# yeyupiaoling/MASR

Measured on AMD Instinct MI355X. Metric: audio-seconds/sec (RTF^-1), conformer_streaming_fbank b32x10s, PCM->fbank->encoder->ctc_greedy->text, higher is better.
Workload: dtype f32; 1 GPU; configs[1]: conformer.yml streaming fbank, batch=32 synthetic 16 kHz 10 s utterances per GPU, ctc_greedy, random-init weights V=4233; global_batch=32, parallelism=dp1, world_size_observed=1, backend=none

## Files before the change

### masr_amd/csrc/common.h

```cpp
#pragma once
#include <hip/hip_runtime.h>
#include <stdint.h>

#include "lm_scorer.h"

#ifndef MASR_EXPERIMENTS
#define MASR_EXPERIMENTS 0
#endif

typedef float f32x4 __attribute__((ext_vector_type(4)));
typedef float f32x16 __attribute__((ext_vector_type(16)));

namespace masr {

struct LdsAttr {
    size_t granted[32] = {};
};
void ensure_dynamic_lds(const void* fn, size_t bytes, LdsAttr& st);
void note_launch_error(const char* what, hipError_t e);

#ifdef __HIPCC__
struct SeqRow {
    int b, t;
};
__device__ __forceinline__ SeqRow seq_row(int b0, int t0, int T, int lr) {
    SeqRow r{b0, t0 + lr};
    while (r.t >= T) {
        r.t -= T;
        ++r.b;
    }
    return r;
}

__device__ __forceinline__ float wave_sum_dpp(float v) {
#define MASR_DPP_F(x, ctrl, rows) \
    __builtin_bit_cast(float, __builtin_amdgcn_update_dpp(0, __builtin_bit_cast(int, (x)), (ctrl), (rows), 0xf, false))
    v += MASR_DPP_F(v, 0x111, 0xf);
    v += MASR_DPP_F(v, 0x112, 0xf);
    v += MASR_DPP_F(v, 0x114, 0xf);
    v += MASR_DPP_F(v, 0x118, 0xf);
    v += MASR_DPP_F(v, 0x142, 0xa);
    v += MASR_DPP_F(v, 0x143, 0xc);
#undef MASR_DPP_F
    return __builtin_bit_cast(float, __builtin_amdgcn_readlane(__builtin_bit_cast(int, v), 63));
}
#endif


enum GemmAct { ACT_NONE = 0, ACT_RELU = 1, ACT_SILU = 2 };
enum GemmAMode { A_PLAIN = 0, A_CONV2 = 1 };
enum GemmEpi { EPI_STD = 0, EPI_GLU = 1, EPI_SPLITK = 2 };

struct GemmArgs {
    const float* A;
    const float* W;
    const float* bias;
    float* C;
    const float* R;
    const int* lens;
    int M, N, K;
    int lda, ldc, ldr;
    int act;
    float alpha;
    int mask_tp;
    int bias_after_alpha;
    int T1, F1, T2, F2, Cc;
    int nsplit, ksplit;
    int skip_rps, skip_div;
    const float* Wp;
};

void launch_gemm(const GemmArgs& a, int amode, int epi, hipStream_t s);
void set_conv2_mid_fill(int pct);
void set_gemm_waves(int n);
void launch_pack_conv2_rows(const float* w, float* p, int K, hipStream_t s);
void launch_gemm_splitk(const GemmArgs& a, float* partial, int nsplit, hipStream_t s, int amode = A_PLAIN);
#if MASR_EXPERIMENTS
bool launch_gemm_bf16x3(const GemmArgs& a, int amode, hipStream_t s);
void set_gemm_bf16x3_waves(int n);
size_t ffn_x3_packed_elems(int dff);
void set_ffn_x3_rotation(int on);
void launch_pack_ffn_x3(const float* w1, const float* w2, unsigned short* p1, unsigned short* p2, int dff, hipStream_t s);
bool launch_ffn_x3(float* x, const float* lnw, const float* lnb, const unsigned short* p1, const float* b1,
                   const unsigned short* p2, const float* b2, int M, int dff, float eps, float scale, hipStream_t s);
#else
inline bool launch_gemm_bf16x3(const GemmArgs&, int, hipStream_t) { return false; }
inline void set_gemm_bf16x3_waves(int) {}
inline size_t ffn_x3_packed_elems(int) { return 0; }
inline void set_ffn_x3_rotation(int) {}
inline void launch_pack_ffn_x3(const float*, const float*, unsigned short*, unsigned short*, int, hipStream_t) {}
inline bool launch_ffn_x3(float*, const float*, const float*, const unsigned short*, const float*, const unsigned short*, const float*,
                          int, int, float, float, hipStream_t) { return false; }
#endif

void launch_layernorm(const float* x, const float* w, const float* b, float* y, int M, float eps,
                      int seq_t, int pad, const int* lens, hipStream_t s);
void set_conv1_nt(int on);
void launch_conv1(const float* feats, const float* mean, const float* istd, const float* w9c, const float* bias,
                  float* out, int B, int T, int F, int C, hipStream_t s);
void launch_dwconv_ln_silu(const float* g, const float* wkc, const float* bias, const float* lnw, const float* lnb,
                           float* out, int nseq, int Tq, int ktaps, float eps, hipStream_t s, const float* gconst = nullptr);
void launch_glu_const(const float* bias512, float* out256, hipStream_t s);
void launch_queue_spin(long long ticks, hipStream_t s);
void launch_queue_nop(hipStream_t s);
void launch_dwconv_bn_silu(const float* g, const float* wkc, const float* bias, const float* scale, const float* shift,
                           float* out, int nseq, int Tq, int ktaps, hipStream_t s, const float* gconst = nullptr);
void launch_dwconv_stride2_ln_silu(const float* g, const float* wkc, const float* bias, const float* lnw,
                                   const float* lnb, float* out, int nseq, int Tin, int ktaps, float eps, hipStream_t s);
void launch_avgpool2(const float* x, float* out, int B, int T, hipStream_t s);
void launch_time_reduce_dw(const float* x, const float* w5c, const float* bias, const int* lens, float* out, int B, int T,
                           int mstride, hipStream_t s);
void launch_recover_add(const float* saved, const float* y, float* x, int B, int T, int L, hipStream_t s);
void launch_softmax_argmax(float* logits, int M, int V, int ldv, int write_probs, int* idx, float* maxp, hipStream_t s);
void launch_ctc_collapse(const int* idx, const float* maxp, const int* nframes, int B, int Tp, int blank,
                         int* tokens, int* ntok, float* score, hipStream_t s);
struct PoolSeg {
    long src, dst;
    int n, pad_;
};
void launch_ctc_collapse_hist(const int* idx, const float* maxp, const int* nframes, const int* in_rows, int ld_in, int B, int Tp,
                              int blank, int* rows, hipStream_t s);
void launch_copy_segments(const float* src, float* dst, const float* src2, float* dst2, const PoolSeg* seg, int nseg,
                          int max_rows, int width, hipStream_t s);
void launch_ctc_collapse_rows(const int* idx, const float* maxp, const int* nframes, int B, int Tp, int blank, int* rows,
                              hipStream_t s);
void launch_topk_prune(const float* probs, int M, int V, int top_n, float cutoff_prob, int* out_idx, float* out_logp,
                       int* out_cnt, int blank, float* out_blank_lp, hipStream_t s);
void launch_argmax_rows(const float* probs, int M, int V, int* idx, float* maxp, hipStream_t s);
// ... 250 lines not shown
```

### masr_amd/csrc/engine.hip

```cpp
#include <math.h>
#include <stdio.h>
#include <stdlib.h>
#include <string.h>

#include <map>
#include <mutex>
#include <string>
#include <vector>

#include "../../include/masr_hip.h"
#include "common.h"

using namespace masr;
namespace masr {
int lm_device_view(masr_lm* lm, LmView* out);
bool lm_word_based(const masr_lm* lm);
}
extern "C" const char* masr_lm_last_error(void);

static thread_local std::string g_err;
static int fail(const std::string& m) {
    g_err = m;
    return 1;
}
// ... 283 lines not shown
    masr_engine* e;
    hipStream_t s;
    bool on;
    ProfScope(masr_engine* e_, hipStream_t s_, int kind, double flops) : e(e_), s(s_) {
        on = e->prof_kind != 0 && (e->prof_kind == kind || (e->prof_kind == PROF_GEMM && (kind == PROF_FFN1 || kind == PROF_CONV2 || kind == PROF_FFN_TAIL || kind == PROF_FFN_HEAD)));
        if (on && e->prof_stride > 1) on = (e->prof_seen++ % e->prof_stride) == 0;
        if (!on) return;
        if (e->prof_used == e->prof_events.size()) {
            hipEvent_t a, b;
            hipEventCreate(&a);
            hipEventCreate(&b);
            e->prof_events.push_back({a, b});
        }
        hipEventRecord(e->prof_events[e->prof_used].first, s);
        e->prof_flops += flops;
    }
    ~ProfScope() {
        if (!on) return;
        hipEventRecord(e->prof_events[e->prof_used].second, s);
        e->prof_used++;
    }
};

struct CallGuard {
    masr_engine* e;
    hipStream_t s;
    size_t n0;
    static size_t packed_count(const masr_engine* e) {
        return e->ffn_packed.size() + e->ffn_dual_packed.size() + e->x3_packed.size() + e->ffn16_packed.size() + e->conv2_packed.size();
    }
    CallGuard(masr_engine* e_, hipStream_t s_) : e(e_), s(s_), n0(packed_count(e_)) {
        if (!e->pack_pending) return;
        if (hipEventQuery(e->pack_ev) == hipSuccess) {
            e->pack_pending = false;
        } else {
            (void)hipGetLastError();
            if ((void*)s != e->pack_stream) (void)hipStreamWaitEvent(s, e->pack_ev, 0);
        }
    }
    ~CallGuard() {
        if (packed_count(e) == n0) return;
        if (!e->pack_ev && hipEventCreateWithFlags(&e->pack_ev, hipEventDisableTiming) != hipSuccess) return;
        if (hipEventRecord(e->pack_ev, s) == hipSuccess) {
            e->pack_stream = (void*)s;
            e->pack_pending = true;
        }
    }
};

static int g_ffn_dual = 0;
static int g_ffn_packed = 2;
static int g_ffn16 = 1;
static int g_conv2_rows = 1;
static int g_bf16x3 = 0;

void gemm(masr_engine* e, hipStream_t s, const float* A, int lda, const float* W, const float* bias, float* C, int ldc,
          int M, int N, int K, int act, float alpha, const float* R, int ldr, int kind = PROF_GEMM,
          const int* lens = nullptr, int mask_tp = 0) {
    GemmArgs a{};
    a.A = A; a.W = W; a.bias = bias; a.C = C; a.R = R; a.lens = lens;
    a.M = M; a.N = N; a.K = K; a.lda = lda; a.ldc = ldc; a.ldr = ldr;
    a.act = act; a.alpha = alpha; a.mask_tp = mask_tp;
    ProfScope ps(e, s, kind, 2.0 * M * (double)N * K);
    if (g_bf16x3 && launch_gemm_bf16x3(a, A_PLAIN, s)) return;
    launch_gemm(a, A_PLAIN, EPI_STD, s);
}

static int g_rowgemm_packed = 1;
const float* packed_rows_of(masr_engine* e, const float* W, int N, hipStream_t s) {
    auto it = e->ffn_packed.find(W);
    if (it == e->ffn_packed.end()) {
        const int Np = (N + 255) / 256 * 256;
        std::pair<DevBuf, DevBuf> pk;
        if (pk.first.ensure((size_t)Np * 256 * sizeof(float))) return nullptr;
        launch_pack_rows_pc(W, pk.first.as<float>(), Np, s, N);
        it = e->ffn_packed.emplace(W, pk).first;
    }
    return it->second.first.as<float>();
}

int packed_ffn_of(masr_engine* e, const float* w1, const float* w2, hipStream_t s, const float** p1, const float** p2) {
    const int d = e->cfg.d_model;
    auto it = e->ffn_packed.find(w1);
    if (it == e->ffn_packed.end()) {
        std::pair<DevBuf, DevBuf> pk;
        CHK(pk.first.ensure((size_t)e->cfg.d_ff * d * sizeof(float)));
        CHK(pk.second.ensure((size_t)e->cfg.d_ff * d * sizeof(float)));
        launch_pack_ffn_pc(w1, w2, pk.first.as<float>(), pk.second.as<float>(), e->cfg.d_ff, s);
        it = e->ffn_packed.emplace(w1, pk).first;
    }
    *p1 = it->second.first.as<float>();
    *p2 = it->second.second.as<float>();
    return 0;
}
static bool sqz_stage_supported(const masr_engine* e) {
    const int K = e->cfg.cnn_kernel;
    return e->cfg.d_model == 256 && e->cfg.d_ff % 128 == 0 && e->cfg.d_ff >= 256 && (K == 31 || K == 15);
}

void rowgemm(masr_engine* e, hipStream_t s, int pro, int epi, const float* A, int lda, const float* lnw,
             const float* lnb, const float* W, const float* bias, float* C, int ldc, int M, int N, const float* R,
             int ldr, float alpha, const int* lens, int mask_tp, int seq_t, int pad, int* out_idx, float* out_maxp,
             int kind = PROF_GEMM, int mstride = 4, int out_seq_t = 0, int out_pad_l = 0, int out_pad_tot = 0,
             int plane_cols = 0, long plane_stride = 0, int a_seq_t = 0, int a_seq_stride = 0, const AttSeq* kv_seqs = nullptr,
             int kv_tq = 0) {
    RowGemmArgs a{};
// ... 601 lines not shown
            std::pair<DevBuf, DevBuf> pk;
            CHK(pk.first.ensure((size_t)dff * d * sizeof(float)));
            CHK(pk.second.ensure((size_t)dff * d * sizeof(float)));
            launch_pack_ffn16(w1, w2, pk.first.as<float>(), pk.second.as<float>(), dff, s);
            it = e->ffn16_packed.emplace(w1, pk).first;
        }
        if (want_tail) {
            ptail = *tail;
            CHK(p16(tail->W, tail->N, &ptail.W));
        }
        if (want_head) {
            phead = *head;
            CHK(p16(head->W, d, &phead.W));
        }
        const int done = launch_ffn16(e->x.as<float>(), lnw, lnb, it->second.first.as<float>(), b1, it->second.second.as<float>(), b2, M,
                                      dff, 1e-5f, scale, s, want_tail ? &ptail : nullptr, want_head ? &phead : nullptr);
        if (done < 0) return fail("ffn(): the 16-row FFN kernel rejected the launch");
        if (want_head && done != 4) return fail("ffn(): head stage was not launched");
        if (tail_done) *tail_done = done == 2;
        if (post_y) launch_layernorm(e->x.as<float>(), post_w, post_b, post_y, M, 1e-5f, 0, 0, nullptr, s);
        return 0;
    }
    if (packed && want_tail && tail->N % 256 == 0) {
        ptail = *tail;
        CHK(packed_rows(tail->W, tail->N, &ptail.W));
        tail = &ptail;
    }
    if (packed && want_head) {
        phead = *head;
        CHK(packed_rows(head->W, d, &phead.W));
        if (split_head) {
            CHK(e->xh.ensure((size_t)M * d * sizeof(float)));
            phead.xout = e->xh.as<float>();
        }
        head = &phead;
    }
    const int done = launch_ffn_fused(e->x.as<float>(), lnw, lnb, kw1, b1, kw2, b2, M, dff, 1e-5f, scale, affine,
                                      nsplit > 1 ? e->ffpart.as<float>() : nullptr, nsplit, s, post_y ? &post : nullptr,
                                      want_tail ? tail : nullptr, want_head ? head : nullptr, packed);
    if (done < 0) return fail("ffn(): launch rejected");
    if (want_head && !(done & 4)) return fail("ffn(): head stage was not launched");
    if (tail_done) *tail_done = done == 2;
    if (post_y && !(done & 1)) launch_layernorm(e->x.as<float>(), post_w, post_b, post_y, M, 1e-5f, 0, 0, nullptr, s);
    return 0;
}

static int g_hot_weights = 0;
static int g_embed_split = 1;
int embed(masr_engine* e, hipStream_t s, const float* feats, int nseq, int T, int* Tq_out, const int* skip_lens = nullptr) {
    const int d = e->cfg.d_model, F = e->cfg.n_mels, F1 = (F - 1) / 2, F2 = (F1 - 1) / 2;
    const int T1 = (T - 1) / 2, Tq = (T1 - 1) / 2;
    if (T < 7 || Tq <= 0) return fail("input too short for Conv2dSubsampling4 (need >= 7 frames)");
    const int M = nseq * Tq;
    CHK(e->x1.ensure((size_t)nseq * T1 * F1 * d * sizeof(float)));
    CHK(e->x2.ensure((size_t)M * F2 * d * sizeof(float)));
    CHK(e->x.ensure((size_t)M * d * sizeof(float)));
    launch_conv1(feats, e->cmvn_mean, e->cmvn_istd, e->conv1_w, e->conv1_b, e->x1.as<float>(), nseq, T, F, d, s);
    {
        GemmArgs a{};
        a.A = e->x1.as<float>(); a.W = e->conv2_w; a.bias = e->conv2_b; a.C = e->x2.as<float>();
        a.M = M * F2; a.N = d; a.K = 9 * d; a.ldc = d; a.act = ACT_RELU; a.alpha = 1.f;
        a.T1 = T1; a.F1 = F1; a.T2 = Tq; a.F2 = F2; a.Cc = d;
        if (skip_lens) { a.lens = skip_lens; a.skip_rps = Tq * F2; a.skip_div = F2; }
        ProfScope ps(e, s, PROF_CONV2, 2.0 * a.M * (double)a.N * a.K);
        const int tiles = ((a.M + 63) / 64) * ((a.N + 63) / 64);
        if (g_bf16x3 && tiles >= 640 && launch_gemm_bf16x3(a, A_CONV2, s)) {
        } else if (tiles < 640) {
            const int nsplit = std::min(8, std::max(2, 1280 / tiles));
            CHK(e->ffpart.ensure((size_t)nsplit * a.M * a.N * sizeof(float)));
            launch_gemm_splitk(a, e->ffpart.as<float>(), nsplit, s, A_CONV2);
        } else {
            if (g_conv2_rows && a.N == 256) {
                auto it = e->conv2_packed.find(e->conv2_w);
                if (it == e->conv2_packed.end()) {
                    std::pair<DevBuf, DevBuf> pk;
                    CHK(pk.first.ensure((size_t)a.N * a.K * sizeof(float)));
                    launch_pack_conv2_rows(e->conv2_w, pk.first.as<float>(), a.K, s);
                    it = e->conv2_packed.emplace(e->conv2_w, pk).first;
                }
                a.Wp = it->second.first.as<float>();
            }
            launch_gemm(a, A_CONV2, EPI_STD, s);
        }
    }
    {
        GemmArgs a{};
        a.A = e->x2.as<float>(); a.lda = F2 * d; a.W = e->embed_w; a.bias = e->embed_b; a.C = e->x.as<float>(); a.ldc = d;
        a.M = M; a.N = d; a.K = F2 * d; a.act = ACT_NONE; a.alpha = sqrtf((float)d);
        a.bias_after_alpha = e->cfg.model_kind == 1 ? 1 : 0;
        if (skip_lens) { a.lens = skip_lens; a.skip_rps = Tq; a.skip_div = 1; }
        ProfScope ps(e, s, PROF_GEMM, 2.0 * M * (double)d * F2 * d);
        const int tiles = ((M + 63) / 64) * ((d + 63) / 64);
        const long wide = (long)((M + 63) / 64) * ((d + 127) / 128);
        const long t128 = (long)((M + 127) / 128) * ((d + 127) / 128);
        if (g_bf16x3 && tiles >= 128 && launch_gemm_bf16x3(a, A_PLAIN, s)) {
        } else if (g_embed_split && tiles >= 128 && t128 >= 100 && t128 <= 128) {
            CHK(e->ffpart.ensure((size_t)4 * M * d * sizeof(float)));
            launch_gemm_splitk(a, e->ffpart.as<float>(), 4, s);
        } else if (g_embed_split && tiles >= 128 && wide >= 200 && wide <= 320) {
            CHK(e->ffpart.ensure((size_t)2 * M * d * sizeof(float)));
            launch_gemm_splitk(a, e->ffpart.as<float>(), 2, s);
        } else if (tiles < 128) {
            const int nsplit = std::min(F2 * d / 32, std::max(2, 256 / tiles));
            CHK(e->ffpart.ensure((size_t)nsplit * M * d * sizeof(float)));
            launch_gemm_splitk(a, e->ffpart.as<float>(), nsplit, s);
        } else {
            launch_gemm(a, A_PLAIN, EPI_STD, s);
        }
    }
    *Tq_out = Tq;
    return 0;
}

int ensure_layer_ws(masr_engine* e, int nseq, int Tq) {
    const int d = e->cfg.d_model, pad = e->cfg.cnn_kernel - 1;
    const size_t M = (size_t)nseq * Tq;
    CHK(e->ln.ensure(M * d * sizeof(float)));
    CHK(e->qkv.ensure(M * 3 * d * sizeof(float)));
    CHK(e->att.ensure(M * d * sizeof(float)));
    CHK(e->lnpad.ensure((size_t)nseq * (Tq + pad) * d * sizeof(float)));
    CHK(e->glu.ensure((size_t)nseq * (Tq + pad) * d * sizeof(float)));
    CHK(e->dwo.ensure(M * d * sizeof(float)));
    return 0;
}

int conv_module(masr_engine* e, hipStream_t s, const LayerW& w, const EncodeCtx& c, bool hist, int K = 0, int mstride = 4,
                bool pw1_done = false, bool pw2_later = false) {
    if (K <= 0) K = e->cfg.cnn_kernel;
    const int d = e->cfg.d_model, pad = K - 1;
    const int M = c.nseq * c.Tq, Mp = c.nseq * (c.Tq + pad);
    float* x = e->x.as<float>();
    if (pw1_done) {
    } else if (hist) {
        launch_layernorm(x, w.ln_conv_w, w.ln_conv_b, e->lnpad.as<float>(), M, 1e-5f, c.Tq, pad, c.lens, s);
        rowgemm(e, s, RG_PRO_PLAIN, RG_EPI_GLU, e->lnpad.as<float>(), d, nullptr, nullptr, w.pw1_w, w.pw1_b,
                e->glu.as<float>(), d, Mp, 2 * d, nullptr, 0, 1.f, nullptr, 0, 0, 0, nullptr, nullptr);
    } else {
        rowgemm(e, s, RG_PRO_LN_PAD, RG_EPI_GLU, x, d, w.ln_conv_w, w.ln_conv_b, w.pw1_w, w.pw1_b, e->glu.as<float>(), d,
                M, 2 * d, nullptr, 0, 1.f, c.lens, 0, c.Tq, 0, nullptr, nullptr, PROF_GEMM, mstride, c.Tq,
                e->cfg.causal ? pad : pad / 2, pad);
    }
    if (pw2_later) return 0;
    const float* gconst = (hist || !e->cfg.causal) ? nullptr : w.gconst;
    {
        RowGemmArgs a{};
        a.A = e->glu.as<float>(); a.lda = d; a.lnw = w.cln_w; a.lnb = w.cln_b; a.dw_w = w.dw_w; a.dw_b = w.dw_b; a.gconst = gconst;
        a.W = w.pw2_w; a.bias = w.pw2_b; a.C = x; a.ldc = d; a.R = x; a.ldr = d; a.M = M; a.N = d; a.alpha = 1.f; a.eps = 1e-5f;
        a.mstride = mstride; a.seq_t = c.Tq; a.pad = pad; a.lens = c.lens; a.mask_tp = c.lens ? c.Tq : 0;
        ProfScope ps(e, s, PROF_GEMM, 2.0 * M * (double)d * d);
// ... 1638 lines not shown
    if (lane == e->lane) return 0;
    EngineWs& active = *e;
    e->parked[e->lane] = active;
    active = e->parked[lane];
    e->parked[lane] = EngineWs();
    e->lane = lane;
    return 0;
}

int masr_side_stream(masr_engine* e, int32_t kind, void** stream_out) {
    if (!e || !stream_out) return fail("null argument");
    if (kind < 0 || kind >= MASR_SIDE_STREAMS)
        return fail("masr_side_stream: kind must be 0 / 1 (prefix search), 2 (preparation), 3 (copy) or 4 (second encoder lane)");
    SideStreams* ss = nullptr;
    if (side_streams_of(e->cfg.device_id, &ss)) return 1;
    *stream_out = (void*)ss->s[kind];
    return 0;
}

int masr_debug_set(masr_engine* e, int32_t key, int32_t value) {
    if (!e) return fail("null engine");
#if !MASR_EXPERIMENTS
    if (value != 0 && (key == 20 || key == 21 || key == 22 || key == 24 || key == 30 || key == 34 || key == 35))
        return fail("masr_debug_set: this key selects an experimental kernel that is not in this build (MASR_BUILD_EXPERIMENTS=1)");
#endif
    if (key == 1) set_ffn_variant(value);
    else if (key == 5) g_no_chain = value;
    else if (key == 6) set_rowgemm_small(value);
    else if (key == 7) set_attention_fewq(value);
    else if (key == 14) set_attention_fold(value);
    else if (key == 15) g_embed_split = value;
    else if (key == 19) g_hot_weights = value;
    else if (key == 20) g_bf16x3 = value;
    else if (key == 21) set_gemm_bf16x3_waves(value);
    else if (key == 22) set_ffn_x3_rotation(value);
    else if (key == 23) g_ffn_packed = value;
    else if (key == 24) g_ffn_dual = value;
    else if (key == 25) g_rowgemm_packed = value;
    else if (key == 26) set_attention_grouped_fold(value);
    else if (key == 27) g_ctc_fused_blocks = value;
    else if (key == 28) set_attention_fewq_wgs(value);
    else if (key == 29) g_few_rows_path = value;
    else if (key == 30) g_split_head = value;
    else if (key == 31) g_efficient_fused = value;
    else if (key == 32) g_beam_lm_cache = value;
    else if (key == 33) set_conv2_mid_fill(value);
    else if (key == 34) g_attn_chain = value;
    else if (key == 35) g_ffn_coop = value;
    else if (key == 36) g_sqz_fused_blocks = value;
    else if (key == 37) g_beam_narrow = value;
    else if (key == 38) e->skip_padding = value;
    else if (key == 39) g_ffn16 = value;
    else if (key == 40) g_conv2_rows = value;
    else if (key == 17) set_gemm_waves(value);
    else if (key == 18) set_conv1_nt(value);
    else if (key == 16) { e->prof_stride = value > 1 ? value : 1; e->prof_seen = 0; }
    else if (key == 8) g_no_ffn_tail = value;
    else if (key == 9) g_no_ffn_head = value;
    else if (key == 12) set_rowgemm_small_blocks(value);
    else if (key == 13) g_ffn_split_blocks = value;
    else if (key == 2) {
        if (value) {
            if (!e->beam_prof) {
                void* p = nullptr;
                HIPCHK(hipMalloc(&p, 16 * sizeof(long long)));
                e->owned.push_back(p);
                e->beam_prof = (long long*)p;
            }
        } else if (e->beam_prof) {
            long long h[16];
            HIPCHK(hipMemcpy(h, e->beam_prof, sizeof(h), hipMemcpyDeviceToHost));
            fprintf(stderr, "beam phases (cycles, last workgroup): setup+hash %lld  extensions %lld  prefixes+count %lld  select %lld  compact %lld\n",
                    h[0], h[1], h[2], h[3], h[4]);
            fprintf(stderr, "  narrow step (%lld frames): tables+candidates %lld  hash+contexts %lld  children+scorer table %lld  extensions %lld  "
                    "prefixes+select %lld  scan %lld  survivors %lld  new prefixes %lld\n", h[5], h[6], h[7], h[8], h[9], h[10], h[11], h[12], h[13]);
            if (h[15] > 0) fprintf(stderr, "  wide step (%lld frames): %.1f distinct scorer contexts per frame\n", h[15], (double)h[14] / (double)h[15]);
            e->beam_prof = nullptr;
        }
    }
    else return fail("unknown debug key");
    return 0;
}

int masr_profile_select(masr_engine* e, int32_t kind) {
    if (!e) return fail("null engine");
    e->prof_kind = kind;
    return 0;
}

int masr_profile_read(masr_engine* e, double* total_ms, int64_t* launches, double* flops, int32_t reset) {
    if (!e) return fail("null engine");
    ENTER(e);
    double tot = 0.0;
    for (size_t i = 0; i < e->prof_used; ++i) {
        HIPCHK(hipEventSynchronize(e->prof_events[i].second));
        float ms = 0.f;
        HIPCHK(hipEventElapsedTime(&ms, e->prof_events[i].first, e->prof_events[i].second));
        tot += ms;
    }
    if (total_ms) *total_ms = tot;
    if (launches) *launches = (int64_t)e->prof_used;
    if (flops) *flops = e->prof_flops;
    if (reset) {
        e->prof_used = 0;
        e->prof_flops = 0.0;
    }
// ... 5 lines not shown
```

### masr_amd/csrc/gemm_f32.hip

```cpp
#include "common.h"

namespace masr {

static constexpr int BK = 32;
static constexpr int LDP = 36;

__device__ __forceinline__ float silu_f(float x) { return x / (1.0f + expf(-x)); }
__device__ __forceinline__ float sigmoid_f(float x) { return 1.0f / (1.0f + expf(-x)); }

template <int BM, int BN, int WM, int WN, int AMODE, int EPI>
__global__ __launch_bounds__(64 * WM * WN) void gemm_f32_kernel(GemmArgs p) {
    static_assert(WM * WN == 4 || WM * WN == 8, "4 or 8 waves");
    constexpr int NT = 64 * WM * WN;
    constexpr int RPP = NT / 8;
    constexpr int TM = BM / WM / 32;
    constexpr int TN = BN / WN / 32;
    constexpr int AL = BM / RPP;
    constexpr int WL = BN / RPP;
    extern __shared__ __align__(16) float smem[];
    float* As = smem;
    float* Ws = smem + 2 * BM * LDP;

    const int tid = threadIdx.x;
    const int lane = tid & 63;
// ... 114 lines not shown
    const int ccol = lane & 31;
    const int rbase = 4 * (lane >> 5);
    if (EPI == EPI_SPLITK) {
        float* cp = p.C + (size_t)blockIdx.y * p.M * p.ldc;
#pragma unroll
        for (int n = 0; n < TN; ++n) {
            const int col = bn + wn * (BN / WN) + n * 32 + ccol;
            if (col >= p.N) continue;
#pragma unroll
            for (int m = 0; m < TM; ++m)
#pragma unroll
                for (int r = 0; r < 16; ++r) {
                    const int row = bm + wm * (BM / WM) + m * 32 + (r & 3) + 8 * (r >> 2) + rbase;
                    if (row < p.M) cp[(size_t)row * p.ldc + col] = acc[m][n][r];
                }
        }
    }
    if (EPI == EPI_STD) {
#pragma unroll
        for (int n = 0; n < TN; ++n) {
            const int col = bn + wn * (BN / WN) + n * 32 + ccol;
            if (col >= p.N) continue;
            const float bv = p.bias ? p.bias[col] : 0.f;
#pragma unroll
            for (int m = 0; m < TM; ++m) {
                float res[16];
#pragma unroll
                for (int r = 0; r < 16; ++r) {
                    const int row = min(bm + wm * (BM / WM) + m * 32 + (r & 3) + 8 * (r >> 2) + rbase, p.M - 1);
                    res[r] = p.R ? p.R[(size_t)row * p.ldr + col] : 0.f;
                }
#pragma unroll
                for (int r = 0; r < 16; ++r) {
                    const int row = bm + wm * (BM / WM) + m * 32 + (r & 3) + 8 * (r >> 2) + rbase;
                    float v = acc[m][n][r] + (p.bias_after_alpha ? 0.f : bv);
                    if (p.act == ACT_RELU) v = fmaxf(v, 0.f);
                    else if (p.act == ACT_SILU) v = silu_f(v);
                    if (p.mask_tp > 0) {
                        const int rc = min(row, p.M - 1);
                        const int b = rc / p.mask_tp, t = rc - b * p.mask_tp;
                        if (4 * t >= p.lens[b]) v = 0.f;
                    }
                    v = res[r] + v * p.alpha + (p.bias_after_alpha ? bv : 0.f);
                    if (row < p.M) p.C[(size_t)row * p.ldc + col] = v;
                }
            }
        }
    }
}

static constexpr int RB_BM = 64;
static constexpr int RB_N = 256;
static constexpr int RB_RING = 8;

__device__ __forceinline__ f32x4 rb_bufld(__amdgpu_buffer_rsrc_t rs, unsigned lane16, unsigned frag) {
    return __builtin_bit_cast(f32x4, __builtin_amdgcn_raw_buffer_load_b128(rs, lane16, frag * 1024u, 0));
}

__global__ __launch_bounds__(512) __attribute__((amdgpu_waves_per_eu(4))) void conv2_rows_kernel(GemmArgs p) {
    __shared__ __align__(16) float As[2][RB_BM * LDP];
    const int tid = threadIdx.x, lane = tid & 63;
    const int wave = __builtin_amdgcn_readfirstlane(tid >> 6);
    const int nbm = (p.M + RB_BM - 1) / RB_BM;
    int bid = blockIdx.x;
    if (p.skip_rps <= 0) {
        const int q = nbm / 8, r = nbm % 8, xcd = bid % 8, idx = bid / 8;
        bid = (xcd < r ? xcd * (q + 1) : r * (q + 1) + (xcd - r) * q) + idx;
    }
    const int bm = bid * RB_BM;
    if (p.skip_rps > 0 && p.lens) {
        const int span = min(bm + RB_BM, p.M) - 1 - bm;
        const int b0 = bm / p.skip_rps, r0 = bm - b0 * p.skip_rps;
        if (r0 + span < p.skip_rps && 4 * (r0 / p.skip_div) >= p.lens[b0]) return;
    }

    const int lrow = tid >> 3, lc4 = (tid & 7) * 4;
    const float* aptr;
    const bool aok = bm + lrow < p.M;
    {
        const int mm = aok ? bm + lrow : 0;
        const int f2 = mm % p.F2, bt = mm / p.F2, t2 = bt % p.T2, b = bt / p.T2;
        aptr = p.A + (((size_t)b * p.T1 + 2 * t2) * p.F1 + 2 * f2) * p.Cc + lc4;
    }
    auto load_a = [&](int kt) -> f32x4 {
        const int cb = kt / 9, pos = kt - 9 * cb;
        const int kh = pos / 3, kw = pos - 3 * kh;
        const size_t aoff = ((size_t)kh * p.F1 + kw) * p.Cc + (size_t)cb * BK;
        return aok ? *reinterpret_cast<const f32x4*>(aptr + aoff) : f32x4{0.f, 0.f, 0.f, 0.f};
    };
    float* const adst = &As[0][lrow * LDP + lc4];

    const int KT = p.K / BK;
    const __amdgpu_buffer_rsrc_t wrs =
        __builtin_amdgcn_make_buffer_rsrc(const_cast<float*>(p.Wp), 0, RB_N * p.K * (int)sizeof(float), 0x00020000);
    const unsigned lane16 = lane * 16;
    const unsigned wfrag0 = (unsigned)(wave * KT) * 4u;
    auto bld = [&](int kt, int g) -> f32x4 { return rb_bufld(wrs, lane16, wfrag0 + (unsigned)min(kt, KT - 1) * 4u + g); };

    f32x4 pre[RB_RING];
#pragma unroll
    for (int i = 0; i < RB_RING; ++i) pre[i] = bld(i >> 2, i & 3);
    f32x16 acc[2];
#pragma unroll
    for (int m = 0; m < 2; ++m)
#pragma unroll
        for (int r = 0; r < 16; ++r) acc[m][r] = 0.f;

    *reinterpret_cast<f32x4*>(adst) = load_a(0);
    __syncthreads();

    const int frow = lane & 31, fcol = (lane >> 5) * 4;
    const float* afrag = &As[0][frow * LDP + fcol];
    for (int kt0 = 0; kt0 < KT; kt0 += 2) {
#pragma unroll
        for (int j = 0; j < 2; ++j) {
            const int kt = kt0 + j;
            if (j == 1 && kt >= KT) break;
            f32x4 areg;
            if (kt + 1 < KT) areg = load_a(kt + 1);
            const float* Ab = afrag + j * RB_BM * LDP;
            f32x4 af[2] = {*reinterpret_cast<const f32x4*>(Ab), *reinterpret_cast<const f32x4*>(Ab + 32 * LDP)};
            __builtin_amdgcn_sched_barrier(0);
#pragma unroll
            for (int g = 0; g < BK / 8; ++g) {
                f32x4 an[2];
                if (g + 1 < BK / 8) {
                    an[0] = *reinterpret_cast<const f32x4*>(Ab + (g + 1) * 8);
                    an[1] = *reinterpret_cast<const f32x4*>(Ab + 32 * LDP + (g + 1) * 8);
                }
                __builtin_amdgcn_sched_barrier(0);
#pragma unroll
                for (int s = 0; s < 4; ++s)
#pragma unroll
                    for (int m = 0; m < 2; ++m)
                        acc[m] = __builtin_amdgcn_mfma_f32_32x32x2f32(af[m][s], pre[4 * j + g][s], acc[m], 0, 0, 0);
                __builtin_amdgcn_sched_barrier(0);
                pre[4 * j + g] = bld(kt + 2, g);
                __builtin_amdgcn_sched_barrier(0);
                if (g + 1 < BK / 8) {
                    af[0] = an[0];
                    af[1] = an[1];
                }
            }
            if (kt + 1 < KT) *reinterpret_cast<f32x4*>(adst + (j ^ 1) * RB_BM * LDP) = areg;
            __syncthreads();
        }
    }

    const int ccol = lane & 31;
    const int rbase = 4 * (lane >> 5);
    const int col = wave * 32 + ccol;
    const float bv = p.bias ? p.bias[col] : 0.f;
#pragma unroll
    for (int m = 0; m < 2; ++m) {
        float res[16];
#pragma unroll
        for (int r = 0; r < 16; ++r) {
            const int row = min(bm + m * 32 + (r & 3) + 8 * (r >> 2) + rbase, p.M - 1);
            res[r] = p.R ? p.R[(size_t)row * p.ldr + col] : 0.f;
        }
#pragma unroll
        for (int r = 0; r < 16; ++r) {
            const int row = bm + m * 32 + (r & 3) + 8 * (r >> 2) + rbase;
            float v = acc[m][r] + (p.bias_after_alpha ? 0.f : bv);
            if (p.act == ACT_RELU) v = fmaxf(v, 0.f);
            else if (p.act == ACT_SILU) v = silu_f(v);
            if (p.mask_tp > 0) {
                const int rc = min(row, p.M - 1);
                const int b = rc / p.mask_tp, t = rc - b * p.mask_tp;
                if (4 * t >= p.lens[b]) v = 0.f;
            }
            v = res[r] + v * p.alpha + (p.bias_after_alpha ? bv : 0.f);
            if (row < p.M) p.C[(size_t)row * p.ldc + col] = v;
        }
    }
}

__global__ __launch_bounds__(256) void pack_conv2_rows_kernel(const float* __restrict__ w, float* __restrict__ p, int K) {
    const size_t e = (size_t)blockIdx.x * 256 + threadIdx.x;
    if (e >= (size_t)RB_N * K) return;
    const int KT = K / BK;
    const int q = (int)(e & 3), lane = (int)((e >> 2) & 63);
    const size_t frag = e >> 8;
    const int g = (int)(frag & 3), kt = (int)((frag >> 2) % KT), wave = (int)((frag >> 2) / KT);
    p[e] = w[(size_t)(32 * wave + (lane & 31)) * K + kt * BK + 8 * g + 4 * (lane >> 5) + q];
}
void launch_pack_conv2_rows(const float* w, float* p, int K, hipStream_t s) {
    const size_t n = (size_t)RB_N * K;
    hipLaunchKernelGGL(pack_conv2_rows_kernel, dim3((unsigned)((n + 255) / 256)), dim3(256), 0, s, w, p, K);
}

static int g_gemm_waves = 8;
static int g_conv2_mid_fill = 50;
void set_conv2_mid_fill(int pct) { g_conv2_mid_fill = pct; }
void set_gemm_waves(int n) { g_gemm_waves = n; }

template <int BM, int BN, int WM, int WN, int AMODE, int EPI>
static void launch_t(const GemmArgs& a, hipStream_t s) {
    const int nbm = (a.M + BM - 1) / BM, nbn = (a.N + BN - 1) / BN;
    const size_t lds = (size_t)2 * (BM + BN) * LDP * sizeof(float);
    auto k = gemm_f32_kernel<BM, BN, WM, WN, AMODE, EPI>;
    static LdsAttr attr;
    ensure_dynamic_lds(reinterpret_cast<const void*>(k), lds, attr);
    hipLaunchKernelGGL(k, dim3(nbm * nbn, EPI == EPI_SPLITK ? a.nsplit : 1), dim3(64 * WM * WN), lds, s, a);
}

__global__ __launch_bounds__(256) void splitk_reduce_kernel(GemmArgs p, const float* __restrict__ partial, float* out) {
    const size_t i = (size_t)blockIdx.x * 256 + threadIdx.x;
    if (i >= (size_t)p.M * p.N) return;
    const int row = (int)(i / p.N), col = (int)(i - (size_t)row * p.N);
    float acc = 0.f;
    for (int sp = 0; sp < p.nsplit; ++sp) acc += partial[((size_t)sp * p.M + row) * p.N + col];
    const float bv = p.bias ? p.bias[col] : 0.f;
    float v = acc + (p.bias_after_alpha ? 0.f : bv);
    if (p.act == ACT_RELU) v = fmaxf(v, 0.f);
    else if (p.act == ACT_SILU) v = silu_f(v);
    const float r = p.R ? p.R[(size_t)row * p.ldr + col] : 0.f;
    out[(size_t)row * p.ldc + col] = r + v * p.alpha + (p.bias_after_alpha ? bv : 0.f);
}

void launch_gemm(const GemmArgs& a, int amode, int epi, hipStream_t s) {
    if (a.M <= 0 || a.N <= 0) return;
    if (amode == A_CONV2 && epi == EPI_SPLITK) {
        launch_t<64, 64, 2, 2, A_CONV2, EPI_SPLITK>(a, s);
        return;
    }
    if (amode == A_CONV2) {
        const long t128c = (long)((a.M + 127) / 128) * ((a.N + 127) / 128);
        const long rounds = (t128c + 511) / 512;
        const bool thin_tail = g_conv2_mid_fill > 0 && t128c >= 200 && t128c <= 1024 &&
                               (t128c - (rounds - 1) * 512) * 100 < (long)g_conv2_mid_fill * 512;
        if (t128c < 200) launch_t<64, 64, 2, 2, A_CONV2, EPI_STD>(a, s);
        else if (thin_tail) launch_t<64, 128, 2, 2, A_CONV2, EPI_STD>(a, s);
        else if (a.Wp && a.N == RB_N && a.K % BK == 0)
            hipLaunchKernelGGL(conv2_rows_kernel, dim3((unsigned)((a.M + RB_BM - 1) / RB_BM)), dim3(512), 0, s, a);
        else if (g_gemm_waves == 8) launch_t<128, 128, 2, 4, A_CONV2, EPI_STD>(a, s);
        else launch_t<128, 128, 2, 2, A_CONV2, EPI_STD>(a, s);
        return;
    }
    if (epi == EPI_SPLITK) {
        if (a.nsplit >= 4 && (long)((a.M + 127) / 128) * ((a.N + 127) / 128) >= 100) launch_t<128, 128, 2, 4, A_PLAIN, EPI_SPLITK>(a, s);
        else if ((long)((a.M + 63) / 64) * ((a.N + 127) / 128) >= 200) launch_t<64, 128, 2, 2, A_PLAIN, EPI_SPLITK>(a, s);
        else launch_t<64, 64, 2, 2, A_PLAIN, EPI_SPLITK>(a, s);
        return;
    }
    const long t128 = (long)((a.M + 127) / 128) * ((a.N + 127) / 128);
    const long t64 = (long)((a.M + 63) / 64) * ((a.N + 127) / 128);
    if (t128 >= 384) launch_t<128, 128, 2, 2, A_PLAIN, EPI_STD>(a, s);
    else if (t64 >= 200) launch_t<64, 128, 2, 2, A_PLAIN, EPI_STD>(a, s);
    else launch_t<64, 64, 2, 2, A_PLAIN, EPI_STD>(a, s);
}

void launch_gemm_splitk(const GemmArgs& a, float* partial, int nsplit, hipStream_t s, int amode) {
    if (a.M <= 0 || a.N <= 0) return;
    GemmArgs b = a;
    const int kts = a.K / BK;
    b.ksplit = (kts + nsplit - 1) / nsplit;
    b.nsplit = (kts + b.ksplit - 1) / b.ksplit;
    b.C = partial;
    b.ldc = a.N;
    launch_gemm(b, amode, EPI_SPLITK, s);
    GemmArgs r = a;
    r.nsplit = b.nsplit;
    hipLaunchKernelGGL(splitk_reduce_kernel, dim3((unsigned)(((size_t)a.M * a.N + 255) / 256)), dim3(256), 0, s, r, partial, a.C);
}

}
```

Before: 51970 audio-seconds/sec.

## Fuse conv1 into conv2 row kernel and reuse row kernel for embed split-K

The conv2 row-streaming kernel gains a fused mode: it computes conv1 (CMVN, 3x3 conv, bias, ReLU) on the fly from the raw fbank features held in LDS, so the large x1 intermediate is never written or read back from global memory. The same kernel gets a plain-A split-K mode, used for the embedding linear layer with a row-packed weight. This removes the x1 round trip and the separate conv1 launch, at the cost of extra per-tile ALU work and LDS use inside the conv2 kernel. Recomputing conv1 per 64-row tile also duplicates overlapping input work.

```diff
diff --git a/masr_amd/csrc/common.h b/masr_amd/csrc/common.h
--- a/masr_amd/csrc/common.h
+++ b/masr_amd/csrc/common.h
@@ -68,12 +68,15 @@
     int nsplit, ksplit;
     int skip_rps, skip_div;
     const float* Wp;
+    const float *feats, *mean, *istd, *c1w, *c1b;
+    int Tin, Fin;
 };
 
 void launch_gemm(const GemmArgs& a, int amode, int epi, hipStream_t s);
 void set_conv2_mid_fill(int pct);
 void set_gemm_waves(int n);
 void launch_pack_conv2_rows(const float* w, float* p, int K, hipStream_t s);
+bool gemm_conv2_rows(const GemmArgs& a);
 void launch_gemm_splitk(const GemmArgs& a, float* partial, int nsplit, hipStream_t s, int amode = A_PLAIN);
 #if MASR_EXPERIMENTS
 bool launch_gemm_bf16x3(const GemmArgs& a, int amode, hipStream_t s);
diff --git a/masr_amd/csrc/engine.hip b/masr_amd/csrc/engine.hip
--- a/masr_amd/csrc/engine.hip
+++ b/masr_amd/csrc/engine.hip
@@ -359,6 +359,8 @@
 static int g_ffn_packed = 2;
 static int g_ffn16 = 1;
 static int g_conv2_rows = 1;
+static int g_conv1_fused = 1;
+static int g_embed_rows = 1;
 static int g_bf16x3 = 0;
 
 void gemm(masr_engine* e, hipStream_t s, const float* A, int lda, const float* W, const float* bias, float* C, int ldc,
@@ -1066,34 +1068,41 @@
     const int T1 = (T - 1) / 2, Tq = (T1 - 1) / 2;
     if (T < 7 || Tq <= 0) return fail("input too short for Conv2dSubsampling4 (need >= 7 frames)");
     const int M = nseq * Tq;
-    CHK(e->x1.ensure((size_t)nseq * T1 * F1 * d * sizeof(float)));
     CHK(e->x2.ensure((size_t)M * F2 * d * sizeof(float)));
     CHK(e->x.ensure((size_t)M * d * sizeof(float)));
-    launch_conv1(feats, e->cmvn_mean, e->cmvn_istd, e->conv1_w, e->conv1_b, e->x1.as<float>(), nseq, T, F, d, s);
     {
         GemmArgs a{};
-        a.A = e->x1.as<float>(); a.W = e->conv2_w; a.bias = e->conv2_b; a.C = e->x2.as<float>();
+        a.W = e->conv2_w; a.bias = e->conv2_b; a.C = e->x2.as<float>();
         a.M = M * F2; a.N = d; a.K = 9 * d; a.ldc = d; a.act = ACT_RELU; a.alpha = 1.f;
         a.T1 = T1; a.F1 = F1; a.T2 = Tq; a.F2 = F2; a.Cc = d;
         if (skip_lens) { a.lens = skip_lens; a.skip_rps = Tq * F2; a.skip_div = F2; }
+        const int tiles = ((a.M + 63) / 64) * ((a.N + 63) / 64);
+        if (tiles >= 640 && g_conv2_rows && a.N == 256) {
+            auto it = e->conv2_packed.find(e->conv2_w);
+            if (it == e->conv2_packed.end()) {
+                std::pair<DevBuf, DevBuf> pk;
+                CHK(pk.first.ensure((size_t)a.N * a.K * sizeof(float)));
+                launch_pack_conv2_rows(e->conv2_w, pk.first.as<float>(), a.K, s);
+                it = e->conv2_packed.emplace(e->conv2_w, pk).first;
+            }
+            a.Wp = it->second.first.as<float>();
+            if (g_conv1_fused && !g_bf16x3 && gemm_conv2_rows(a)) {
+                a.feats = feats; a.mean = e->cmvn_mean; a.istd = e->cmvn_istd; a.c1w = e->conv1_w; a.c1b = e->conv1_b;
+                a.Tin = T; a.Fin = F;
+            }
+        }
+        if (!a.feats) {
+            CHK(e->x1.ensure((size_t)nseq * T1 * F1 * d * sizeof(float)));
+            launch_conv1(feats, e->cmvn_mean, e->cmvn_istd, e->conv1_w, e->conv1_b, e->x1.as<float>(), nseq, T, F, d, s);
+            a.A = e->x1.as<float>();
+        }
         ProfScope ps(e, s, PROF_CONV2, 2.0 * a.M * (double)a.N * a.K);
-        const int tiles = ((a.M + 63) / 64) * ((a.N + 63) / 64);
         if (g_bf16x3 && tiles >= 640 && launch_gemm_bf16x3(a, A_CONV2, s)) {
         } else if (tiles < 640) {
             const int nsplit = std::min(8, std::max(2, 1280 / tiles));
             CHK(e->ffpart.ensure((size_t)nsplit * a.M * a.N * sizeof(float)));
             launch_gemm_splitk(a, e->ffpart.as<float>(), nsplit, s, A_CONV2);
         } else {
-            if (g_conv2_rows && a.N == 256) {
-                auto it = e->conv2_packed.find(e->conv2_w);
-                if (it == e->conv2_packed.end()) {
-                    std::pair<DevBuf, DevBuf> pk;
-                    CHK(pk.first.ensure((size_t)a.N * a.K * sizeof(float)));
-                    launch_pack_conv2_rows(e->conv2_w, pk.first.as<float>(), a.K, s);
-                    it = e->conv2_packed.emplace(e->conv2_w, pk).first;
-                }
-                a.Wp = it->second.first.as<float>();
-            }
             launch_gemm(a, A_CONV2, EPI_STD, s);
         }
     }
@@ -1109,6 +1118,16 @@
         const long t128 = (long)((M + 127) / 128) * ((d + 127) / 128);
         if (g_bf16x3 && tiles >= 128 && launch_gemm_bf16x3(a, A_PLAIN, s)) {
         } else if (g_embed_split && tiles >= 128 && t128 >= 100 && t128 <= 128) {
+            if (g_embed_rows && d == 256 && (F2 * d) % 32 == 0) {
+                auto it = e->conv2_packed.find(e->embed_w);
+                if (it == e->conv2_packed.end()) {
+                    std::pair<DevBuf, DevBuf> pk;
+                    CHK(pk.first.ensure((size_t)a.N * a.K * sizeof(float)));
+                    launch_pack_conv2_rows(e->embed_w, pk.first.as<float>(), a.K, s);
+                    it = e->conv2_packed.emplace(e->embed_w, pk).first;
+                }
+                a.Wp = it->second.first.as<float>();
+            }
             CHK(e->ffpart.ensure((size_t)4 * M * d * sizeof(float)));
             launch_gemm_splitk(a, e->ffpart.as<float>(), 4, s);
         } else if (g_embed_split && tiles >= 128 && wide >= 200 && wide <= 320) {
@@ -2853,6 +2872,8 @@
     else if (key == 38) e->skip_padding = value;
     else if (key == 39) g_ffn16 = value;
     else if (key == 40) g_conv2_rows = value;
+    else if (key == 41) g_conv1_fused = value;
+    else if (key == 42) g_embed_rows = value;
     else if (key == 17) set_gemm_waves(value);
     else if (key == 18) set_conv1_nt(value);
     else if (key == 16) { e->prof_stride = value > 1 ? value : 1; e->prof_seen = 0; }
diff --git a/masr_amd/csrc/gemm_f32.hip b/masr_amd/csrc/gemm_f32.hip
--- a/masr_amd/csrc/gemm_f32.hip
+++ b/masr_amd/csrc/gemm_f32.hip
@@ -190,13 +190,20 @@
 static constexpr int RB_BM = 64;
 static constexpr int RB_N = 256;
 static constexpr int RB_RING = 8;
+static constexpr int RB_PP = 49;
+enum { RB_X1 = 0, RB_FUSED = 1, RB_PLAIN = 2 };
 
 __device__ __forceinline__ f32x4 rb_bufld(__amdgpu_buffer_rsrc_t rs, unsigned lane16, unsigned frag) {
     return __builtin_bit_cast(f32x4, __builtin_amdgcn_raw_buffer_load_b128(rs, lane16, frag * 1024u, 0));
 }
 
+__device__ constexpr int rb_tap(int g) { return g == 0 ? 0 : g == 1 ? 2 : g == 2 ? 4 : g == 3 ? 6 : 9; }
+
+template <int AM>
 __global__ __launch_bounds__(512) __attribute__((amdgpu_waves_per_eu(4))) void conv2_rows_kernel(GemmArgs p) {
+    constexpr int XS = AM == RB_FUSED ? 10 * RB_N + RB_BM * RB_PP : 4;
     __shared__ __align__(16) float As[2][RB_BM * LDP];
+    __shared__ __align__(16) float Xs[XS];
     const int tid = threadIdx.x, lane = tid & 63;
     const int wave = __builtin_amdgcn_readfirstlane(tid >> 6);
     const int nbm = (p.M + RB_BM - 1) / RB_BM;
@@ -211,24 +218,33 @@
         const int b0 = bm / p.skip_rps, r0 = bm - b0 * p.skip_rps;
         if (r0 + span < p.skip_rps && 4 * (r0 / p.skip_div) >= p.lens[b0]) return;
     }
+    const int KT = p.K / BK;
+    const int kt_lo = AM == RB_PLAIN ? (int)blockIdx.y * p.ksplit : 0;
+    const int kt_hi = AM == RB_PLAIN ? min(kt_lo + p.ksplit, KT) : KT;
 
     const int lrow = tid >> 3, lc4 = (tid & 7) * 4;
-    const float* aptr;
+    const float* aptr = nullptr;
     const bool aok = bm + lrow < p.M;
-    {
+    if (AM == RB_X1) {
         const int mm = aok ? bm + lrow : 0;
         const int f2 = mm % p.F2, bt = mm / p.F2, t2 = bt % p.T2, b = bt / p.T2;
         aptr = p.A + (((size_t)b * p.T1 + 2 * t2) * p.F1 + 2 * f2) * p.Cc + lc4;
+    } else if (AM == RB_PLAIN) {
+        aptr = p.A + (size_t)(aok ? bm + lrow : 0) * p.lda + lc4;
     }
     auto load_a = [&](int kt) -> f32x4 {
-        const int cb = kt / 9, pos = kt - 9 * cb;
-        const int kh = pos / 3, kw = pos - 3 * kh;
-        const size_t aoff = ((size_t)kh * p.F1 + kw) * p.Cc + (size_t)cb * BK;
+        size_t aoff;
+        if (AM == RB_PLAIN) {
+            aoff = (size_t)kt * BK;
+        } else {
+            const int cb = kt / 9, pos = kt - 9 * cb;
+            const int kh = pos / 3, kw = pos - 3 * kh;
+            aoff = ((size_t)kh * p.F1 + kw) * p.Cc + (size_t)cb * BK;
+        }
         return aok ? *reinterpret_cast<const f32x4*>(aptr + aoff) : f32x4{0.f, 0.f, 0.f, 0.f};
     };
     float* const adst = &As[0][lrow * LDP + lc4];
 
-    const int KT = p.K / BK;
     const __amdgpu_buffer_rsrc_t wrs =
         __builtin_amdgcn_make_buffer_rsrc(const_cast<float*>(p.Wp), 0, RB_N * p.K * (int)sizeof(float), 0x00020000);
     const unsigned lane16 = lane * 16;
@@ -237,25 +253,71 @@
 
     f32x4 pre[RB_RING];
 #pragma unroll
-    for (int i = 0; i < RB_RING; ++i) pre[i] = bld(i >> 2, i & 3);
+    for (int i = 0; i < RB_RING; ++i) pre[i] = bld(kt_lo + (i >> 2), i & 3);
+    __builtin_amdgcn_sched_barrier(0);
+
+    const float* const w1s = Xs;
+    const float* const xrow = Xs + 10 * RB_N + lrow * RB_PP;
+    if (AM == RB_FUSED) {
+        for (int i = tid; i < 9 * RB_N; i += 512) Xs[i] = p.c1w[i];
+        if (tid < RB_N) Xs[9 * RB_N + tid] = p.c1b[tid];
+        const int m = min(bm + lrow, p.M - 1);
+        const int f2 = m % p.F2, bt = m / p.F2, t2 = bt % p.T2, b = bt / p.T2;
+        const float* src = p.feats + ((size_t)b * p.Tin + 4 * t2) * p.Fin + 4 * f2;
+        for (int q = tid & 7; q < RB_PP; q += 8) {
+            const int dt = q / 7, df = q - 7 * dt, f = 4 * f2 + df;
+            Xs[10 * RB_N + lrow * RB_PP + q] = (src[dt * p.Fin + df] - p.mean[f]) * p.istd[f];
+        }
+    }
+    auto c1_rd = [&](int kt, int t, f32x4& w, float& x) {
+        const int cb = kt / 9, pos = kt - 9 * cb, kh = pos / 3, kw = pos - 3 * kh;
+        x = xrow[2 * kh * 7 + 2 * kw + (t / 3) * 7 + t % 3];
+        w = *reinterpret_cast<const f32x4*>(w1s + t * RB_N + 32 * cb + lc4);
+    };
+    auto c1_fma = [&](f32x4& c, const f32x4& w, float x) {
+#pragma unroll
+        for (int q = 0; q < 4; ++q) c[q] = fmaf(w[q], x, c[q]);
+    };
+    auto c1_bias = [&](int kt) -> f32x4 { return *reinterpret_cast<const f32x4*>(w1s + 9 * RB_N + 32 * (kt / 9) + lc4); };
+    auto c1_relu = [&](f32x4& c) {
+#pragma unroll
+        for (int q = 0; q < 4; ++q) c[q] = fmaxf(c[q], 0.f);
+    };
+
+    if (AM == RB_FUSED) {
+        __syncthreads();
+        f32x4 c = c1_bias(0);
+#pragma unroll
+        for (int t = 0; t < 9; ++t) {
+            f32x4 w;
+            float x;
+            c1_rd(0, t, w, x);
+            c1_fma(c, w, x);
+        }
+        c1_relu(c);
+        *reinterpret_cast<f32x4*>(adst) = c;
+    }
     f32x16 acc[2];
 #pragma unroll
     for (int m = 0; m < 2; ++m)
 #pragma unroll
         for (int r = 0; r < 16; ++r) acc[m][r] = 0.f;
 
-    *reinterpret_cast<f32x4*>(adst) = load_a(0);
+    if (AM != RB_FUSED) *reinterpret_cast<f32x4*>(adst) = load_a(kt_lo);
     __syncthreads();
 
     const int frow = lane & 31, fcol = (lane >> 5) * 4;
     const float* afrag = &As[0][frow * LDP + fcol];
-    for (int kt0 = 0; kt0 < KT; kt0 += 2) {
+    for (int kt0 = kt_lo; kt0 < kt_hi; kt0 += 2) {
 #pragma unroll
         for (int j = 0; j < 2; ++j) {
             const int kt = kt0 + j;
-            if (j == 1 && kt >= KT) break;
+            if (j == 1 && kt >= kt_hi) break;
+            const bool next = kt + 1 < kt_hi;
+            const int ktn = min(kt + 1, kt_hi - 1);
             f32x4 areg;
-            if (kt + 1 < KT) areg = load_a(kt + 1);
+            if (AM == RB_FUSED) areg = c1_bias(ktn);
+            else if (next) areg = load_a(kt + 1);
             const float* Ab = afrag + j * RB_BM * LDP;
             f32x4 af[2] = {*reinterpret_cast<const f32x4*>(Ab), *reinterpret_cast<const f32x4*>(Ab + 32 * LDP)};
             __builtin_amdgcn_sched_barrier(0);
@@ -266,6 +328,13 @@
                     an[0] = *reinterpret_cast<const f32x4*>(Ab + (g + 1) * 8);
                     an[1] = *reinterpret_cast<const f32x4*>(Ab + 32 * LDP + (g + 1) * 8);
                 }
+                constexpr int NTAP = 3;
+                f32x4 cw[NTAP];
+                float cx[NTAP];
+                if (AM == RB_FUSED) {
+#pragma unroll
+                    for (int t = rb_tap(g); t < rb_tap(g + 1); ++t) c1_rd(ktn, t, cw[t - rb_tap(g)], cx[t - rb_tap(g)]);
+                }
                 __builtin_amdgcn_sched_barrier(0);
 #pragma unroll
                 for (int s = 0; s < 4; ++s)
@@ -275,12 +344,17 @@
                 __builtin_amdgcn_sched_barrier(0);
                 pre[4 * j + g] = bld(kt + 2, g);
                 __builtin_amdgcn_sched_barrier(0);
+                if (AM == RB_FUSED) {
+#pragma unroll
+                    for (int t = rb_tap(g); t < rb_tap(g + 1); ++t) c1_fma(areg, cw[t - rb_tap(g)], cx[t - rb_tap(g)]);
+                }
                 if (g + 1 < BK / 8) {
                     af[0] = an[0];
                     af[1] = an[1];
                 }
             }
-            if (kt + 1 < KT) *reinterpret_cast<f32x4*>(adst + (j ^ 1) * RB_BM * LDP) = areg;
+            if (AM == RB_FUSED) c1_relu(areg);
+            if (next) *reinterpret_cast<f32x4*>(adst + (j ^ 1) * RB_BM * LDP) = areg;
             __syncthreads();
         }
     }
@@ -288,6 +362,17 @@
     const int ccol = lane & 31;
     const int rbase = 4 * (lane >> 5);
     const int col = wave * 32 + ccol;
+    if (AM == RB_PLAIN) {
+        float* cp = p.C + (size_t)blockIdx.y * p.M * p.ldc;
+#pragma unroll
+        for (int m = 0; m < 2; ++m)
+#pragma unroll
+            for (int r = 0; r < 16; ++r) {
+                const int row = bm + m * 32 + (r & 3) + 8 * (r >> 2) + rbase;
+                if (row < p.M) cp[(size_t)row * p.ldc + col] = acc[m][r];
+            }
+        return;
+    }
     const float bv = p.bias ? p.bias[col] : 0.f;
 #pragma unroll
     for (int m = 0; m < 2; ++m) {
@@ -357,6 +442,17 @@
     out[(size_t)row * p.ldc + col] = r + v * p.alpha + (p.bias_after_alpha ? bv : 0.f);
 }
 
+static int conv2_tiles(const GemmArgs& a) {
+    const long t128c = (long)((a.M + 127) / 128) * ((a.N + 127) / 128);
+    const long rounds = (t128c + 511) / 512;
+    const bool thin_tail = g_conv2_mid_fill > 0 && t128c >= 200 && t128c <= 1024 &&
+                           (t128c - (rounds - 1) * 512) * 100 < (long)g_conv2_mid_fill * 512;
+    if (t128c < 200) return 64;
+    if (thin_tail) return 128;
+    return a.Wp && a.N == RB_N && a.K % BK == 0 ? 0 : 256;
+}
+bool gemm_conv2_rows(const GemmArgs& a) { return a.M > 0 && conv2_tiles(a) == 0; }
+
 void launch_gemm(const GemmArgs& a, int amode, int epi, hipStream_t s) {
     if (a.M <= 0 || a.N <= 0) return;
     if (amode == A_CONV2 && epi == EPI_SPLITK) {
@@ -364,19 +460,23 @@
         return;
     }
     if (amode == A_CONV2) {
-        const long t128c = (long)((a.M + 127) / 128) * ((a.N + 127) / 128);
-        const long rounds = (t128c + 511) / 512;
-        const bool thin_tail = g_conv2_mid_fill > 0 && t128c >= 200 && t128c <= 1024 &&
-                               (t128c - (rounds - 1) * 512) * 100 < (long)g_conv2_mid_fill * 512;
-        if (t128c < 200) launch_t<64, 64, 2, 2, A_CONV2, EPI_STD>(a, s);
-        else if (thin_tail) launch_t<64, 128, 2, 2, A_CONV2, EPI_STD>(a, s);
-        else if (a.Wp && a.N == RB_N && a.K % BK == 0)
-            hipLaunchKernelGGL(conv2_rows_kernel, dim3((unsigned)((a.M + RB_BM - 1) / RB_BM)), dim3(512), 0, s, a);
-        else if (g_gemm_waves == 8) launch_t<128, 128, 2, 4, A_CONV2, EPI_STD>(a, s);
+        const int tiles = conv2_tiles(a);
+        if (tiles == 64) launch_t<64, 64, 2, 2, A_CONV2, EPI_STD>(a, s);
+        else if (tiles == 128) launch_t<64, 128, 2, 2, A_CONV2, EPI_STD>(a, s);
+        else if (a.Wp && a.N == RB_N && a.K % BK == 0) {
+            const dim3 grid((unsigned)((a.M + RB_BM - 1) / RB_BM));
+            if (a.feats) hipLaunchKernelGGL(conv2_rows_kernel<RB_FUSED>, grid, dim3(512), 0, s, a);
+            else hipLaunchKernelGGL(conv2_rows_kernel<RB_X1>, grid, dim3(512), 0, s, a);
+        } else if (g_gemm_waves == 8) launch_t<128, 128, 2, 4, A_CONV2, EPI_STD>(a, s);
         else launch_t<128, 128, 2, 2, A_CONV2, EPI_STD>(a, s);
         return;
     }
     if (epi == EPI_SPLITK) {
+        if (a.Wp && a.N == RB_N && a.K % BK == 0) {
+            hipLaunchKernelGGL(conv2_rows_kernel<RB_PLAIN>, dim3((unsigned)((a.M + RB_BM - 1) / RB_BM), (unsigned)a.nsplit), dim3(512),
+                               0, s, a);
+            return;
+        }
         if (a.nsplit >= 4 && (long)((a.M + 127) / 128) * ((a.N + 127) / 128) >= 100) launch_t<128, 128, 2, 4, A_PLAIN, EPI_SPLITK>(a, s);
         else if ((long)((a.M + 63) / 64) * ((a.N + 127) / 128) >= 200) launch_t<64, 128, 2, 2, A_PLAIN, EPI_SPLITK>(a, s);
         else launch_t<64, 64, 2, 2, A_PLAIN, EPI_SPLITK>(a, s);
```

Result: faster. 53020 audio-seconds/sec (median of 6 runs) (+2.0%).
